# MingruiYuan/SpoofSV

Hardware: AMD Instinct MI355X
Metric: mel-frames/sec (Text2Mel+SSRN train) (higher is better)
Workload: dtype f32 (conv GEMMs: fp32 operands scaled by a power of two and split into fp16 hi+lo = 22 significand bits, three exact fp16 MFMAs per product, fp32 accumulate: ~2^-22 per product, gradients within 3e-6 of float64 = the exact-fp32 path's level); 1 GPU; train_text2mel + train_ssrn (train/ordinary.py step: fwd, l1+bin-div+guided-att losses, bwd, Adam), batch 32 utterances/GPU, N=186, T=325, 80 mel -> 513x1300 linear, hidden 256, random-init; global_batch=32, parallelism=dp1, launch=hipGraph replay, ddp=none

## Files before the change

### spoofsv_amd/csrc/api_conv.hip

```cpp
#include "ssv_host.h"

int conv_shifts(int k, int dilation, int causal, int* shift) {
  SSV_CHECK(k == 1 || k == 3, SSV_UNSUPPORTED, "conv1d: kernel_size %d not supported (1 or 3)", k);
  SSV_CHECK(dilation >= 1 && dilation * (k - 1) <= 54, SSV_UNSUPPORTED, "conv1d: dilation %d not supported (k=%d)", dilation, k);
  const int j0 = causal ? k - 1 : (k - 1) / 2;
  for (int j = 0; j < 3; ++j) shift[j] = j < k ? (j - j0) * dilation : 0;
  return 0;
}
extern "C" int ssv_conv_shifts(int k, int dilation, int causal, int* shift3) { return conv_shifts(k, dilation, causal, shift3); }

int amax_of(const float* x, long x_bs, int B, long n_item, const float* given, int ngiven, float* fb, AmaxList* out, hipStream_t st) {
  if (given) {
    SSV_CHECK(ngiven > 0, SSV_BAD_SHAPE, "operand scale list given with %d entries per item", ngiven);
    out->p = given; out->n = ngiven;
    return 0;
  }
  SSV_CHECK(fb, SSV_BAD_SHAPE, "split-fp16: no operand scales given and no workspace to compute them in");
  SSV_CHECK(B <= SSV_AMAX_FB_FLOATS, SSV_UNSUPPORTED, "split-fp16: batch %d needs caller-provided operand scales (ssv_absmax)", B);
  int npb = SSV_AMAX_FB_FLOATS / B;
  if (npb > 64) npb = 64;
  const long pieces = (n_item + 4095) / 4096;
  if (npb > pieces) npb = (int)(pieces > 0 ? pieces : 1);
  SSV_TRY(ssv_launch_absmax(x, x_bs, B, n_item, fb, npb, st));
  out->p = fb; out->n = npb;
// ... 194 lines not shown
  l.fb_dy = t.take(AMAX_FB_BYTES);
  l.fb_x = t.take(AMAX_FB_BYTES);
  l.total = t.off;
  return l;
}
extern "C" size_t ssv_conv1d_bwd_weight_workspace(int B, int Cin, int Cout, int L, int k) { return wgrad_ws(B, Cin, Cout, L, k).total; }
int conv1d_bwd_weight_impl(const float* dy, long dy_bs, const float* x, long x_bs, float* dw, int B, int Cin, int Cout, int L, int k, int dilation,
                           int causal, void* ws, size_t ws_bytes, ssv_stream_t stream, const float* part, float* pgrads, int n2, int nblk,
                           const float* dy_amax, int dy_namax, const float* x_amax, int x_namax) {
  SSV_CHECK(dy && x && dw && B > 0 && Cin > 0 && Cout > 0 && L > 0, SSV_BAD_SHAPE, "conv1d_bwd_weight: bad argument");
  const WgradWs l = wgrad_ws(B, Cin, Cout, L, k);
  SSV_CHECK(ws && ws_bytes >= l.total, SSV_BAD_SHAPE, "conv1d_bwd_weight: workspace too small");
  hipStream_t st = (hipStream_t)stream;
  GemmNT g;
  SSV_TRY(conv_shifts(k, dilation, causal, g.shift));
  int Z = l.Z;
  const float* slabs = ws_f32(ws, l.slabs);
  const long n = (long)Cout * Cin * k;
  g.A = dy; g.sab = dy_bs; g.sam = L; g.La = L;
  g.X = x; g.sxb = x_bs; g.sxc = L; g.Lx = L;
  g.M = Cout; g.Nc = Cin; g.KT = k; g.B = B;
  const bool bf3 = wgrad_bf3_runs(B, Cout, Cin, L, dy_bs, x_bs);
  if (!bf3 && Z > B) Z = B;
  if (Z == 1) { g.C = dw; g.scz = n; g.scm = (long)Cin * k; g.scc = k; g.scj = 1; }
  else { g.C = ws_f32(ws, l.slabs); g.scz = n; g.scm = (long)Cin * k; g.scc = 1; g.scj = Cin; }
  g.Z = Z; g.bstep = Z;
  if (bf3) {
    if (k != 3 && ssv_nt_bf3_xrow(1, Cout, Cin)) g.bstep = 0;
    if (use_f16()) {
      AmaxList la, lx;
      SSV_TRY(amax_of(dy, dy_bs, B, (long)Cout * L, dy_amax, dy_namax, ws_f32(ws, l.fb_dy), &la, st));
      SSV_TRY(amax_of(x, x_bs, B, (long)Cin * L, x_amax, x_namax, ws_f32(ws, l.fb_x), &lx, st));
      g.f16 = 1; g.a_amax = la.p; g.a_namax = la.n * B; g.x_amax = lx.p; g.x_namax = lx.n * B;
    }
    SSV_TRY(ssv_launch_gemm_nt_bf3(g, st));
  } else if (L == 1 && k == 1) {
    SSV_TRY(ssv_launch_linear_len1_wgrad(dy, dy_bs, x, x_bs, dw, B, Cin, Cout, st));
    if (part) SSV_TRY(ssv_reduce_partial_rows(part, pgrads, n2, nblk, st));
    return 0;
  } else SSV_TRY(ssv_launch_gemm_nt(g, st));
  if (part) {
    if (Z > 1 && nblk <= 768) return ssv_launch_reduce_pair(slabs, dw, Cout, Cin, k, Z, part, pgrads, n2, nblk, st);
    SSV_TRY(ssv_reduce_partial_rows(part, pgrads, n2, nblk, st));
  }
  if (Z > 1) SSV_TRY(ssv_launch_reduce_slabs_perm(slabs, dw, Cout, Cin, k, Z, st));
  return 0;
}
extern "C" int ssv_conv1d_bwd_weight(const float* dy, long dy_bs, const float* dy_amax, int dy_namax, const float* x, long x_bs, const float* x_amax, int x_namax,
                                     float* dw, int B, int Cin, int Cout, int L, int k, int dilation, int causal,
                                     void* ws, size_t ws_bytes, ssv_stream_t stream) {
  return conv1d_bwd_weight_impl(dy, dy_bs, x, x_bs, dw, B, Cin, Cout, L, k, dilation, causal, ws, ws_bytes, stream, nullptr, nullptr, 0, 0,
                                dy_amax, dy_namax, x_amax, x_namax);
}

extern "C" int ssv_conv1d_bwd_weight_multi_ok(int B, int Cin, int Cout, int L, int k) {
  return (k == 1 || k == 3) && L >= 8 && wgrad_bf3_runs_dense(B, Cout, Cin, L) ? 1 : 0;
}
extern "C" int ssv_conv1d_bwd_weight_multi_splits(int njobs, int B, int Cin, int Cout, int L, int k) {
  const int kt = k == 3 ? 3 : 1;
  if (njobs < 1) njobs = 1;
  const long tiles = (long)ssv_nt_bf3_tiles(kt, Cout, Cin) * njobs;
  if (kt == 1 && ssv_nt_bf3_xrow(1, Cout, Cin)) return xrow_slabs(tiles, B, L);
  int z = nt_slabs(tiles, njobs, B, L, kt, Cout, Cin);
  if (z > B) z = B;
  if (z < 1) z = 1;
  return z;
}
extern "C" size_t ssv_conv1d_bwd_weight_multi_workspace(int njobs, int B, int Cin, int Cout, int L, int k) {
  return align256((size_t)njobs * ssv_conv1d_bwd_weight_multi_splits(njobs, B, Cin, Cout, L, k) * Cout * Cin * k * sizeof(float));
}
extern "C" int ssv_conv1d_bwd_weight_multi(const ssv_wgrad_job* jobs_dev, int njobs, long dy_bs, long x_bs, int B, int Cin, int Cout, int L, int k, int max_shift,
                                           int n2, int nblk, void* ws, size_t ws_bytes, ssv_stream_t stream) {
  SSV_CHECK(jobs_dev && njobs > 0 && B > 0 && Cin > 0 && Cout > 0 && L > 0, SSV_BAD_SHAPE, "conv1d_bwd_weight_multi: bad argument");
  SSV_CHECK(ssv_conv1d_bwd_weight_multi_ok(B, Cin, Cout, L, k), SSV_UNSUPPORTED, "conv1d_bwd_weight_multi: shape or arithmetic mode not supported");
  SSV_CHECK(n2 == 0 || nblk <= 768, SSV_UNSUPPORTED, "conv1d_bwd_weight_multi: %d partial rows (max 768)", nblk);
  SSV_CHECK(ws && ws_bytes >= ssv_conv1d_bwd_weight_multi_workspace(njobs, B, Cin, Cout, L, k), SSV_BAD_SHAPE, "conv1d_bwd_weight_multi: workspace too small");
  hipStream_t st = (hipStream_t)stream;
  const int Z = ssv_conv1d_bwd_weight_multi_splits(njobs, B, Cin, Cout, L, k);
  const long n = (long)Cout * Cin * k;
  GemmNT g;
  g.sab = dy_bs; g.sam = L; g.La = L;
  g.sxb = x_bs; g.sxc = L; g.Lx = L;
  g.C = (float*)ws; g.scz = n; g.scm = (long)Cin * k; g.scc = 1; g.scj = Cin;
  g.M = Cout; g.Nc = Cin; g.KT = k; g.B = B; g.Z = Z; g.bstep = (k != 3 && ssv_nt_bf3_xrow(1, Cout, Cin)) ? 0 : Z;
  g.jobs = jobs_dev; g.njobs = njobs; g.max_shift = max_shift;
  g.f16 = use_f16() ? 1 : 0;
  SSV_TRY(ssv_launch_gemm_nt_bf3(g, st));
  return ssv_launch_reduce_pair_multi(jobs_dev, njobs, (const float*)ws, Cout, Cin, k, Z, n2, nblk, st);
}

static ConvWs deconv_fwd_ws(int Cin, int Cout) { return conv_ws(2 * split_bytes(Cout, Cin, 2)); }
extern "C" size_t ssv_deconv1d_k2s2_fwd_workspace(int Cin, int Cout) { return deconv_fwd_ws(Cin, Cout).total; }
extern "C" int ssv_deconv1d_k2s2_fwd(const float* x, long x_bs, const float* x_amax, int x_namax, const float* w, const void* w_packed, const float* bias,
                                     float* y, long y_bs, float* y_amax, int y_namax, int B, int Cin, int Cout, int L, void* ws, size_t ws_bytes, ssv_stream_t stream) {
  SSV_CHECK(x && w && y && B > 0 && Cin > 0 && Cout > 0 && L > 0, SSV_BAD_SHAPE, "deconv1d_k2s2_fwd: bad argument");
  SSV_CHECK(!y_amax || y_namax > 0, SSV_BAD_SHAPE, "deconv1d_k2s2_fwd: scale list of %d entries", y_namax);
  hipStream_t st = (hipStream_t)stream;
  if (use_bf3(B, L, Cin, Cout)) {
    const ConvWs l = deconv_fwd_ws(Cin, Cout);
    SSV_CHECK(ws && ws_bytes >= l.total, SSV_BAD_SHAPE, "deconv1d_k2s2_fwd: workspace too small");
    const int M2 = 2 * Cout, Kpad = pad32(Cin);
    const bool f16 = use_f16();
    float* aux = ws_f32(ws, l.aux);
    SplitPlanes pl = packed_planes(w_packed, Cin, M2, 1).tr;
    if (!pl.hi) {
      pl.hi = ws_u16(ws, l.main); pl.lo = ws_u16(ws, l.main + split_bytes(M2, Cin, 1));
      if (f16) { SSV_TRY(ssv_launch_pack_split_f16(w, (long)Cin * M2, pl.hi, pl.lo, M2, Cin, Kpad, 1, 1, (long)M2, 1, aux, st)); pl.inv = aux + 64; }
      else SSV_TRY(ssv_launch_pack_split(w, pl.hi, pl.lo, M2, Cin, Kpad, 1, 1, (long)M2, 1, 0, st));
    }
    GemmNNB g;
    if (f16) {
// ... 102 lines not shown
```

### spoofsv_amd/csrc/misc.hip

```cpp
#include "ssv_common.h"
#include "../../include/ssv_hip.h"

__global__ __launch_bounds__(256) void reduce_slabs_kernel(const float* __restrict__ s, float* __restrict__ out, long n, int Z, long stride) {
  const long i = (long)blockIdx.x * 256 + threadIdx.x;
  if (i >= n) return;
  float a[4] = {0.f, 0.f, 0.f, 0.f};
  int z = 0;
  for (; z + 3 < Z; z += 4) {
#pragma unroll
    for (int u = 0; u < 4; ++u) a[u] += s[(long)(z + u) * stride + i];
  }
  for (; z < Z; ++z) a[0] += s[(long)z * stride + i];
  out[i] = (a[0] + a[1]) + (a[2] + a[3]);
}
int ssv_launch_reduce_slabs(const float* slabs, float* out, long n, int Z, long stride, hipStream_t st) {
  hipLaunchKernelGGL(reduce_slabs_kernel, dim3(ssv_cdiv(n, 256)), dim3(256), 0, st, slabs, out, n, Z, stride);
  return ssv_check_launch("reduce_slabs");
}

__device__ __forceinline__ void reduce_perm_block(const float* __restrict__ s, float* __restrict__ out, int Nc, int KT, long n, int Z, int block,
                                                  float* __restrict__ stage ) {
  const long P = n / KT;
  const long q = (long)block * 256 + threadIdx.x;
  if (KT == 1) {
// ... 101 lines not shown
  __shared__ float red[8][32];
  const ssv_wgrad_job jb = jobs[blockIdx.y];
  const float* __restrict__ s = slabs + (long)blockIdx.y * Z * n;
  __shared__ __attribute__((aligned(16))) float stage[256 * 3];
  if ((int)blockIdx.x < nA) {
    reduce_perm_block(s, jb.dw, Nc, KT, n, Z, (int)blockIdx.x, stage);
    return;
  }
  if (!jb.part) return;
  const __attribute__((address_space(1))) float* __restrict__ part = (const __attribute__((address_space(1))) float*)jb.part;
  const int li = threadIdx.x & 31, rg = threadIdx.x >> 5;
  const int i = ((int)blockIdx.x - nA) * 32 + li;
  red[rg][li] = i < n2 ? ssv_fold_rows(part, n2, nblk, i, rg) : 0.f;
  __syncthreads();
  if (rg == 0 && i < n2) {
    float t = 0.f;
#pragma unroll
    for (int r = 0; r < 8; ++r) t += red[r][li];
    jb.pgrads[i] = t;
  }
}
int ssv_launch_reduce_pair_multi(const ssv_wgrad_job* jobs, int njobs, const float* slabs, int M, int Nc, int KT, int Z, int n2, int nblk, hipStream_t st) {
  const long n = (long)M * Nc * KT;
  const int nA = ssv_cdiv((long)M * Nc, 256), nB = n2 > 0 ? ssv_cdiv(n2, 32) : 0;
  hipLaunchKernelGGL(reduce_pair_multi_kernel, dim3(nA + nB, njobs), dim3(256), 0, st, jobs, slabs, Nc, KT, n, Z, nA, n2, nblk);
  return ssv_check_launch("reduce_pair_multi");
}

__global__ __launch_bounds__(256) void pack_wt_kernel(const float* __restrict__ w, float* __restrict__ wt, int Cout, int Cin, int KT) {
  const long i = (long)blockIdx.x * 256 + threadIdx.x;
  const long n = (long)Cout * Cin * KT;
  if (i >= n) return;
  const int j = (int)(i % KT);
  const long r = i / KT;
  const int o = (int)(r % Cout), c = (int)(r / Cout);
  wt[i] = w[((long)o * Cin + c) * KT + j];
}
int ssv_launch_pack_wt(const float* w, float* wt, int Cout, int Cin, int KT, hipStream_t st) {
  const long n = (long)Cout * Cin * KT;
  hipLaunchKernelGGL(pack_wt_kernel, dim3(ssv_cdiv(n, 256)), dim3(256), 0, st, w, wt, Cout, Cin, KT);
  return ssv_check_launch("pack_wt");
}

__global__ __launch_bounds__(256) void linear_len1_fwd_kernel(const float* __restrict__ x, long x_bs, const float* __restrict__ w, const float* __restrict__ bias,
                                                              const float* __restrict__ bias_b, long sbb, float* __restrict__ y, long y_bs, int B, int K, int M) {
  const long t = ((long)blockIdx.x * 256 + threadIdx.x) >> 3;
  const int j = threadIdx.x & 7;
// ... 579 lines not shown
```

### spoofsv_amd/csrc/ssv_common.h

```cpp
#pragma once
#include <hip/hip_runtime.h>
#include <stdint.h>
#include <stddef.h>
#include "../../include/ssv_hip.h"

int ssv_fail(int code, const char* fmt, ...);
#define SSV_BAD_SHAPE (-1)
#define SSV_UNSUPPORTED (-2)
#define SSV_CHECK(cond, code, ...) do { if (!(cond)) return ssv_fail((code), __VA_ARGS__); } while (0)
#define SSV_TRY(expr) do { int _e = (expr); if (_e) return _e; } while (0)
int ssv_check_launch(const char* what);

typedef __attribute__((ext_vector_type(4))) float f32x4;

struct GemmNN {
  const float* A = nullptr; long sab = 0, sam = 0, sac = 0, saj = 0;
  const float* X = nullptr; long sxb = 0, sxc = 0, sxn = 1; int Lx = 0;
  float* C = nullptr; long scb = 0, scm = 0, scn = 1;
  const float* bias = nullptr;
  const float* bias_b = nullptr; long sbb = 0;
  const float* R = nullptr; long srb = 0, srm = 0, srn = 1;
  int M = 0, N = 0, Kc = 0, KT = 1, B = 1;
  int shift[3] = {0, 0, 0};
  float alpha = 1.f;
// ... 21 lines not shown
  const float* R = nullptr; long srb = 0, srm = 0;
  int M = 0, N = 0, Kc = 0, KT = 1, B = 1;
  int shift[3] = {0, 0, 0};
  int sxn = 1, scn = 1;
  int row_pair = 0; float* c_amax = nullptr; int c_namax = 0;
  unsigned short* hs_planes = nullptr; long hs_plane_bytes = 0; int hs_npad = 0;
  int hs_keep_h = 1;
  int ksplit = 1; long scz = 0; int skip_rows = 0;
  const unsigned short* x0_planes = nullptr; const float* x0_amax = nullptr; int xsplit0 = 0;
  int perm_h = 0, epi = 0, first = 0;
  float* cstate = nullptr;
  float* lstm_out = nullptr; int lstm_s = 0, lstm_lo = 0, lstm_D = 0, xsplit = 0; long sab = 0;
  const unsigned short* A0hi = nullptr; const unsigned short* A0lo = nullptr;
  float* gates_out = nullptr;
  int f16 = 0; const float* a_inv = nullptr; const float* x_amax = nullptr; int x_namax = 0; long x_amax_bs = 0;
  float* colstats = nullptr;
  const float* xrow_w = nullptr; long xrow_sk = 0;
};
int ssv_launch_gemm_nn_bf3(const GemmNNB& g, hipStream_t st);
int ssv_launch_gemm_pwln(const GemmNNB& g, const float* gamma, const float* beta, float* y, long ybs, float* stats, float* y_amax, int namax, int act,
                         hipStream_t st);
int ssv_launch_gemm_nt_bf3(const GemmNT& g, hipStream_t st);
int ssv_launch_gemm_nt3r(const GemmNT& g, dim3 grid, int mtiles, int tchunks, int ring_ms, hipStream_t st);
struct PwLnBw {
  const float* dy; long dy_bs; const float* pre; const float* stats; const float* gamma; const float* beta;
  float* dpre; float* part; int part_rows; int part_q; float* amax; int namax;
  const unsigned short* Ahi; const unsigned short* Alo; const float* a_inv;
  float* dx; long dx_bs; const float* xrow_w; long xrow_sk;
  int M, Cin, L, act;
};
bool ssv_pwln_bwd_fused_ok(int B, int Cin, int Cout, int L);
int ssv_launch_pwln_bwd(const PwLnBw& q, int B, int f16, hipStream_t st);
bool ssv_nt_bf3_xrow(int KT, int M, int Nc);
bool ssv_nt_bf3_fits(const GemmNT& g);
int ssv_launch_pack_split(const float* w, void* hi, void* lo, int M, int K, int Kpad, int KT, long sm, long sk, long sj, int perm_h, hipStream_t st,
                          int nch_total = 0, int ch_off = 0);
int ssv_launch_pack_split_f16(const float* w, long w_elems, void* hi, void* lo, int M, int K, int Kpad, int KT, long sm, long sk, long sj, float* aux, hipStream_t st);
int ssv_launch_pack_split_f16_list(const float* w, void* hi, void* lo, int M, int K, int Kpad, int KT, long sm, long sk, long sj, int perm_h,
                                   const float* list, int nlist, float* inv_out, hipStream_t st, int nch_total = 0, int ch_off = 0);
#define SSV_F16_AUX_FLOATS 128
#define SSV_AMAX_FALLBACK 64
int ssv_launch_absmax(const float* x, long x_bs, int B, long n, float* out, int npb, hipStream_t st);
int ssv_nt_bf3_tiles(int KT, int M, int Nc);
void ssv_nt_bf3_tile(int KT, int M, int Nc, int* wm, int* ntc);
int ssv_nt_bf3_wg_per_cu(int KT, int wm, int ntc);
int ssv_precision();
// ... 97 lines not shown
```

### spoofsv_amd/csrc/wgrad_nt.hip

```cpp
#include "bf3_common.h"

#ifdef SSV_NT_STAMP
__device__ unsigned long long ssv_nt_stamps[64];
__device__ unsigned long long ssv_nt_wg[4096 * 4];
extern "C" int ssv_debug_nt_wg(unsigned long long* out) { return (int)hipMemcpyFromSymbol(out, HIP_SYMBOL(ssv_nt_wg), sizeof(ssv_nt_wg)); }
#define NT_WG(k, v) do { const unsigned w_ = blockIdx.z * gridDim.x + blockIdx.x; if (threadIdx.x == 0 && w_ < 4096u) ssv_nt_wg[w_ * 4 + (k)] = (v); } while (0)
#define NT_STAMP(k) do { if (stamp_on && (unsigned)(stamp_s - 24) < 8u) ssv_nt_stamps[(stamp_s - 24) * 8 + (k)] = __builtin_readcyclecounter(); } while (0)
extern "C" int ssv_debug_nt_stamps(unsigned long long* out) { return (int)hipMemcpyFromSymbol(out, HIP_SYMBOL(ssv_nt_stamps), sizeof(ssv_nt_stamps)); }
#else
#define NT_STAMP(k) do {} while (0)
#define NT_WG(k, v) do {} while (0)
#endif
constexpr int NT_FD = 1;
template <int KT, int WM, int NTC, int F16, int XR = 0, int WV = 4>
__global__ __launch_bounds__(64 * WV, WV == 4 ? 2 : 1) void gemm_nt_bf3_kernel(const GemmNT p, const int mtiles) {
  constexpr int NTH = 64 * WV;
  constexpr int KB = 64, KG = KB / 8, KS = KB / 32;
  constexpr int NCH = 16 * NTC;
  constexpr int X_SLOTS = KG * NCH;
  constexpr int NX = X_SLOTS / NTH;
  static_assert(X_SLOTS % NTH == 0, "tile slots must be a multiple of the workgroup size");
  __shared__ uint4 lds[2][2 * X_SLOTS];
  __shared__ float amax_sm[2 * WV];

// ... 353 lines not shown
}
int ssv_nt_bf3_wg_per_cu(int KT, int wm, int ntc) {
  if (wm == 4) return 1;
  if (KT == 3) return wm == 2 ? 2 : (ntc >= 4 ? 3 : 4);
  if (wm == 2) return ntc >= 6 ? 2 : 3;
  return ntc >= 6 ? 3 : (ntc >= 4 ? 4 : 5);
}
int ssv_nt_bf3_tiles(int KT, int M, int Nc) {
  int wm, ntc;
  ssv_nt_bf3_tile(KT, M, Nc, &wm, &ntc);
  return ssv_cdiv(ssv_nt_bf3_xrow(KT, M, Nc) ? M - 1 : M, 64 * wm) * ssv_cdiv(Nc, 16 * ntc);
}
bool ssv_nt_bf3_xrow(int KT, int M, int Nc) {
  int wm, ntc;
  ssv_nt_bf3_tile(KT, M, Nc, &wm, &ntc);
  return KT == 1 && wm == 2 && ntc == 6 && M > 128 && M % 128 == 1;
}

bool ssv_nt_bf3_fits(const GemmNT& g) {
  const long lim = 1L << 30;
  return (long)(g.B - 1) * g.sab + (long)(g.M - 1) * g.sam + g.La < lim && (long)(g.B - 1) * g.sxb + (long)(g.Nc - 1) * g.sxc + g.Lx < lim &&
         (long)g.B * g.sab < lim && (long)g.B * g.sxb < lim && g.La >= 8 && g.Lx >= 8;
}
int ssv_launch_gemm_nt_bf3(const GemmNT& g, hipStream_t st) {
  SSV_CHECK(g.M > 0 && g.Nc > 0 && g.La > 0 && g.B > 0 && g.Z > 0 && g.bstep >= 0, SSV_BAD_SHAPE, "gemm_nt_bf3: empty problem");
  SSV_CHECK(g.KT == 1 || g.KT == 3, SSV_UNSUPPORTED, "gemm_nt_bf3: kernel_size %d", g.KT);
  SSV_CHECK(g.sat == 1 && g.sxn == 1, SSV_UNSUPPORTED, "gemm_nt_bf3: rows must be contiguous in time");
  SSV_CHECK(g.Z <= 65535, SSV_UNSUPPORTED, "gemm_nt_bf3: Z=%d exceeds grid.z", g.Z);
  SSV_CHECK(ssv_nt_bf3_fits(g), SSV_UNSUPPORTED, "gemm_nt_bf3: an operand spans 2^30 elements or more");
  int wm, ntc;
  ssv_nt_bf3_tile(g.KT, g.M, g.Nc, &wm, &ntc);
  const bool xr = ssv_nt_bf3_xrow(g.KT, g.M, g.Nc);
  SSV_CHECK(g.bstep > 0 || xr, SSV_UNSUPPORTED, "gemm_nt_bf3: range slabs are built for the extra-row kernel only");
  const int mtiles = ssv_cdiv(xr ? g.M - 1 : g.M, 64 * wm);
  const int nz = g.jobs ? g.njobs * g.Z : g.Z;
  SSV_CHECK(nz <= 65535, SSV_UNSUPPORTED, "gemm_nt_bf3: %d slabs exceed grid.z", nz);
  const dim3 grid(mtiles * ssv_cdiv(g.Nc, 16 * ntc), 1, nz);
  SSV_CHECK(!g.f16 || g.jobs || (g.a_amax && g.x_amax && g.a_namax > 0 && g.x_namax > 0), SSV_BAD_SHAPE, "gemm_nt_bf3: split-fp16 needs both operand scales");
  int ring_ms = -1;
  if (g.KT == 3 && wm == 2 && ntc == 4) {
    ring_ms = g.max_shift;
    if (!g.jobs) { ring_ms = 0; for (int j = 0; j < 3; ++j) ring_ms = abs(g.shift[j]) > ring_ms ? abs(g.shift[j]) : ring_ms; }
    if (ring_ms > 64) ring_ms = -1;
  }
  if (ssv_shape_log_on()) {
    char nm[96], note[96];
    const int nj = g.jobs ? g.njobs : 1;
    if (ring_ms >= 0) snprintf(nm, sizeof nm, "gemm_nt3r_kernel<%d, %d>", wm, g.f16);
    else if (wm == 4) snprintf(nm, sizeof nm, "gemm_nt_bf3_kernel<%d, 2, %d, %d, 0, 8>", g.KT, ntc, g.f16);
    else snprintf(nm, sizeof nm, "gemm_nt_bf3_kernel<%d, %d, %d, %d, %d, 4>", g.KT, wm, ntc, g.f16, xr ? 1 : 0);
    snprintf(note, sizeof note, "jobs=%d B=%d M=%d Nc=%d L=%d k=%d Z=%d", nj, g.B, g.M, g.Nc, g.La, g.KT, g.Z);
    ssv_shape_log(nm, grid, dim3(wm == 4 ? 512 : 256), 2.0 * nj * g.B * g.M * g.Nc * g.La * g.KT,
                  4.0 * nj * ((double)g.B * g.M * g.La + (double)g.B * g.Nc * g.Lx + (double)g.Z * g.M * g.Nc * g.KT), note);
  }
  if (ring_ms >= 0) {
    const int tchunks = ssv_cdiv((g.La > g.Lx ? g.La : g.Lx) + ring_ms, 64);
    return ssv_launch_gemm_nt3r(g, grid, mtiles, tchunks, ring_ms, st);
  }
  if (xr) {
    if (g.f16) hipLaunchKernelGGL((gemm_nt_bf3_kernel<1, 2, 6, 1, 1>), grid, dim3(256), 0, st, g, mtiles);
    else hipLaunchKernelGGL((gemm_nt_bf3_kernel<1, 2, 6, 0, 1>), grid, dim3(256), 0, st, g, mtiles);
    return ssv_check_launch("gemm_nt_bf3 (extra row)");
  }
  if (g.KT == 1 && wm == 4 && ntc == 8) {
    if (g.f16) hipLaunchKernelGGL((gemm_nt_bf3_kernel<1, 2, 8, 1, 0, 8>), grid, dim3(512), 0, st, g, mtiles);
    else hipLaunchKernelGGL((gemm_nt_bf3_kernel<1, 2, 8, 0, 0, 8>), grid, dim3(512), 0, st, g, mtiles);
    return ssv_check_launch("gemm_nt_bf3 (8 waves)");
  }
#define SSV_NT(K_, A_, C_) if (g.KT == K_ && wm == A_ && ntc == C_) { \
    if (g.f16) hipLaunchKernelGGL((gemm_nt_bf3_kernel<K_, A_, C_, 1>), grid, dim3(256), 0, st, g, mtiles); \
    else hipLaunchKernelGGL((gemm_nt_bf3_kernel<K_, A_, C_, 0>), grid, dim3(256), 0, st, g, mtiles); \
    return ssv_check_launch("gemm_nt_bf3"); }
  SSV_NT(3, 2, 4)
  SSV_NT(1, 2, 8) SSV_NT(1, 2, 6) SSV_NT(1, 2, 2) SSV_NT(1, 1, 4)
#undef SSV_NT
  return ssv_fail(SSV_UNSUPPORTED, "gemm_nt_bf3: no tile %d,%d for kernel size %d", wm, ntc, g.KT);
// ... 3 lines not shown
```

### spoofsv_amd/csrc/wgrad_nt3r.hip

```cpp
#include "bf3_common.h"

#ifdef SSV_NT_STAMP
__device__ unsigned long long ssv_nt3r_stamps[64];
__device__ unsigned long long ssv_nt3r_wg[4096 * 4];
extern "C" int ssv_debug_nt3r_wg(unsigned long long* out) { return (int)hipMemcpyFromSymbol(out, HIP_SYMBOL(ssv_nt3r_wg), sizeof(ssv_nt3r_wg)); }
extern "C" int ssv_debug_nt3r_stamps(unsigned long long* out) { return (int)hipMemcpyFromSymbol(out, HIP_SYMBOL(ssv_nt3r_stamps), sizeof(ssv_nt3r_stamps)); }
#define NT_WG(k, v) do { const unsigned w_ = blockIdx.z * gridDim.x + blockIdx.x; if (threadIdx.x == 0 && w_ < 4096u) ssv_nt3r_wg[w_ * 4 + (k)] = (v); } while (0)
#define NT_STAMP(k) do { if (stamp_on && (unsigned)(stamp_s - 24) < 8u) ssv_nt3r_stamps[(stamp_s - 24) * 8 + (k)] = __builtin_readcyclecounter(); } while (0)
#else
#define NT_STAMP(k) do {} while (0)
#define NT_WG(k, v) do {} while (0)
#endif
typedef short ssv_s4 __attribute__((ext_vector_type(4)));
typedef __attribute__((address_space(3))) ssv_s4 ssv_lds_s4;
typedef unsigned ssv_u2 __attribute__((ext_vector_type(2)));
typedef __attribute__((address_space(3))) ssv_u2 ssv_lds_u2;
__device__ __forceinline__ void ssv_lds_store2(unsigned addr, unsigned a, unsigned b) {
#if defined(__HIP_DEVICE_COMPILE__)
  *(ssv_lds_u2*)(size_t)addr = (ssv_u2){a, b};
#else
  (void)addr; (void)a; (void)b;
#endif
}
__device__ __forceinline__ uint2 ssv_lds_read_tr16(unsigned addr) {
#if defined(__HIP_DEVICE_COMPILE__)
  return __builtin_bit_cast(uint2, __builtin_amdgcn_ds_read_tr16_b64_v4i16((ssv_lds_s4*)(size_t)addr));
#else
  (void)addr; return make_uint2(0u, 0u);
#endif
}
template <int WM, int F16>
__global__ __launch_bounds__(256, 2) void gemm_nt3r_kernel(const GemmNT p, const int mtiles, const int tchunks, const int max_shift) {
  constexpr int KT = 3, NTC = 4, NCH = 64, KB = 64, KS = 2;
  constexpr int R_FD = 1;
  constexpr unsigned ROWB = 128, PLANE = 288 * ROWB;
  __shared__ __attribute__((aligned(16))) unsigned char ring[2 * PLANE];
  __shared__ float amax_sm[8];

  const int tid = threadIdx.x, lane = tid & 63, wave = tid >> 6;
  NT_WG(0, __builtin_amdgcn_s_memrealtime()); NT_WG(2, __builtin_readcyclecounter());
  const unsigned wg = ssv_xcd_order(blockIdx.x + gridDim.x * blockIdx.z, gridDim.x * gridDim.z);
  const int bxx = (int)(wg % gridDim.x);
  int z = (int)(wg / gridDim.x);
  const float* __restrict__ Ap = p.A;
  const float* __restrict__ Xp = p.X;
  float* __restrict__ Cp = p.C;
  int shj[3] = {p.shift[0], p.shift[1], p.shift[2]};
  const float* __restrict__ a_amax = p.a_amax;
  const float* __restrict__ x_amax = p.x_amax;
  int a_namax = p.a_namax, x_namax = p.x_namax;
  if (p.jobs) {
    const int job = z / p.Z;
    z -= job * p.Z;
    const ssv_wgrad_job* __restrict__ jb = p.jobs + job;
    Ap = ssv_global(jb->dy); Xp = ssv_global(jb->x); Cp = p.C + (long)job * p.Z * p.scz;
    shj[0] = jb->shift[0]; shj[1] = jb->shift[1]; shj[2] = jb->shift[2];
    a_amax = ssv_global(jb->dy_amax); x_amax = ssv_global(jb->x_amax); a_namax = jb->dy_namax; x_namax = jb->x_namax;
  }
  float as = 1.f, xs = 1.f, us = 1.f;
  if constexpr (F16) {
    float sa, sx, ia, ix;
    ssv_pow2_scale(ssv_list_max<4>(a_amax, a_namax, amax_sm), sa, ia);
    ssv_pow2_scale(ssv_list_max<4>(x_amax, x_namax, amax_sm + 4), sx, ix);
    as = ssv_uniform(sa); xs = ssv_uniform(sx);
    us = ssv_uniform(ia * ix);
  }
  const int mt = bxx % mtiles, ct = bxx / mtiles;
  const int m0 = mt * 64 * WM, c0 = ct * NCH;
  const int kq = lane >> 4, nq = lane & 15;

  f32x4 acc[WM][KT][NTC];
#pragma unroll
  for (int i = 0; i < WM; ++i)
#pragma unroll
    for (int j = 0; j < KT; ++j)
#pragma unroll
      for (int q = 0; q < NTC; ++q) acc[i][j][q] = (f32x4){0.f, 0.f, 0.f, 0.f};

  uint4 AH[2][WM][KS], AL[2][WM][KS];
  uint4 rx[4];

  const __amdgpu_buffer_rsrc_t rsA = __builtin_amdgcn_make_buffer_rsrc(const_cast<float*>(Ap), 0,
      (int)(((long)(p.B - 1) * p.sab + (long)(p.M - 1) * p.sam + p.La) * 4), 0x00020000);
  const __amdgpu_buffer_rsrc_t rsX = __builtin_amdgcn_make_buffer_rsrc(const_cast<float*>(Xp), 0,
      (int)(((long)(p.B - 1) * p.sxb + (long)(p.Nc - 1) * p.sxc + p.Lx) * 4), 0x00020000);
  const unsigned arow = (unsigned)(((m0 + wave * WM * 16 + nq) * (int)p.sam + 4 * kq) * 4);
  const unsigned a16 = 16u * (unsigned)p.sam * 4u;
  const int cq = lane >> 4, tq = lane & 15;
  const unsigned xrow = (unsigned)(((c0 + 16 * wave + 4 * cq) * (int)p.sxc + 4 * tq) * 4);
  const unsigned x1 = (unsigned)p.sxc * 4u;
  const bool rows_in_c = c0 + NCH <= p.Nc;
  const unsigned ringb = (unsigned)(size_t)(__attribute__((address_space(3))) unsigned char*)ring;
  const unsigned waddr = ringb + (unsigned)(4 * tq) * ROWB + (unsigned)((wave ^ ((tq & 1) | (((tq >> 2) & 1) << 1))) << 5) + (unsigned)cq * 8u;
  const int q4 = (lane >> 2) & 3, pp = lane & 3;
  int lrow[2];
  lrow[0] = 4 * kq + (q4 >> 1) + 16 * (q4 & 1);
  lrow[1] = lrow[0] + 2;
  unsigned lbase[2], key5[KT][2];
#pragma unroll
  for (int r = 0; r < 2; ++r) {
    lbase[r] = ringb + (unsigned)lrow[r] * ROWB + (unsigned)pp * 8u;
#pragma unroll
    for (int j = 0; j < KT; ++j) { const int rr = shj[j] + lrow[r]; key5[j][r] = (unsigned)(((rr >> 2) & 1) | (((rr >> 4) & 1) << 1)) << 5; }
  }

  const int nb = (p.B - z + p.bstep - 1) / p.bstep;
  const int total = nb * tchunks;
  int cb[4], ct0[4];
  cb[0] = z; ct0[0] = 0;
  auto next_chunk = [&](int b, int t0, int& nb_, int& nt0) __attribute__((always_inline)) {
    nt0 = t0 + KB; nb_ = b;
    if (nt0 >= tchunks * KB) { nt0 = 0; nb_ = b + p.bstep; }
  };
#pragma unroll
  for (int k = 1; k < 4; ++k) next_chunk(cb[k - 1], ct0[k - 1], cb[k], ct0[k]);

  auto loadA = [&](auto set, int b, int t0) __attribute__((always_inline)) {
    constexpr int SET = decltype(set)::value;
    const unsigned so = ((unsigned)b * (unsigned)p.sab + (unsigned)t0) * 4u;
#pragma unroll
    for (int i = 0; i < WM; ++i)
#pragma unroll
      for (int s2 = 0; s2 < KS; ++s2) {
        AH[SET][i][s2] = __builtin_bit_cast(uint4, __builtin_amdgcn_raw_buffer_load_b128(rsA, (int)(arow + (so + i * a16)) + s2 * 128, 0, 0));
        AL[SET][i][s2] = __builtin_bit_cast(uint4, __builtin_amdgcn_raw_buffer_load_b128(rsA, (int)(arow + (so + i * a16)) + s2 * 128 + 64, 0, 0));
      }
  };
  auto loadA1 = [&](auto set, int b, int t0, int idx) __attribute__((always_inline)) {
    constexpr int SET = decltype(set)::value;
    const unsigned so = ((unsigned)b * (unsigned)p.sab + (unsigned)t0) * 4u;
// ... 70 lines not shown
    const int stamp_s = n + 16;
#endif
    NT_STAMP(0);
#pragma unroll
    for (int j = 0; j < KT; ++j) {
      constexpr int G = KS * NTC;
      uint4 fb[R_FD + 1][2];
      unsigned su[KS];
#pragma unroll
      for (int s2 = 0; s2 < KS; ++s2) su[s2] = (unsigned)((64 * n + shj[j] + 32 * s2) & 255) * ROWB;
      auto frag = [&](int g, uint4 (&f)[2]) __attribute__((always_inline)) {
        const int s2 = g / NTC, cbk = g % NTC;
        const unsigned a0 = lbase[0] + su[s2] + ((unsigned)(cbk << 5) ^ key5[j][0]);
        const unsigned a1 = lbase[1] + su[s2] + ((unsigned)(cbk << 5) ^ key5[j][1]);
        const uint2 h0u = ssv_lds_read_tr16(a0), h1u = ssv_lds_read_tr16(a1);
        const uint2 l0u = ssv_lds_read_tr16(a0 + PLANE), l1u = ssv_lds_read_tr16(a1 + PLANE);
        f[0] = make_uint4(h0u.x, h0u.y, h1u.x, h1u.y);
        f[1] = make_uint4(l0u.x, l0u.y, l1u.x, l1u.y);
      };
#pragma unroll
      for (int g = 0; g < R_FD; ++g) frag(g, fb[g]);
#pragma unroll
      for (int g = 0; g < G; ++g) {
        if (g + R_FD < G) frag(g + R_FD, fb[(g + R_FD) % (R_FD + 1)]);
        if (j == 0 && g < 4 * WM) loadA1(NXT{}, cb[1], ct0[1], g);
        if (j == 1 && g < 4) loadX1(cb[3], ct0[3], g);
        __builtin_amdgcn_sched_barrier(0);
        const int s2 = g / NTC, q = g % NTC;
        if (ct0[0] + 32 * s2 >= p.La) continue;
        const uint4 bh = fb[g % (R_FD + 1)][0];
        const uint4 bl = fb[g % (R_FD + 1)][1];
#pragma unroll
        for (int i = 0; i < WM; ++i) {
          const uint4 a_h = AH[CUR::value][i][s2];
          const uint4 a_l = AL[CUR::value][i][s2];
          acc[i][j][q] = mma16<F16>(a_l, bh, acc[i][j][q]);
          acc[i][j][q] = mma16<F16>(a_h, bl, acc[i][j][q]);
          acc[i][j][q] = mma16<F16>(a_h, bh, acc[i][j][q]);
        }
      }
      if (j == 0) {
        NT_STAMP(2);
        commitX((n + 2) & 3, ct0[2]);
        NT_STAMP(3);
      }
      if (j == 1) NT_STAMP(5);
// ... 4 lines not shown
      }
    }
    __syncthreads();
#pragma unroll
    for (int k = 0; k < 3; ++k) { cb[k] = cb[k + 1]; ct0[k] = ct0[k + 1]; }
    next_chunk(cb[2], ct0[2], cb[3], ct0[3]);
  };

  if (total > 0) {
    loadA(P0{}, cb[0], ct0[0]);
    loadX(cb[0], ct0[0]);
    {
#pragma unroll
      for (int i = 0; i < 4; ++i) {
        ssv_lds_store2(waddr + 3u * 64u * ROWB + i * ROWB, 0u, 0u);
        ssv_lds_store2(waddr + 3u * 64u * ROWB + i * ROWB + PLANE, 0u, 0u);
      }
    }
    commitX(0, ct0[0]);
    loadX(cb[1], ct0[1]);
    splitA(P0{}, ct0[0]);
    commitX(1, ct0[1]);
    loadX(cb[2], ct0[2]);
    __syncthreads();
    int n = 0;
    for (; n + 1 < total; n += 2) {
      chunk(P0{}, n);
      chunk(P1{}, n + 1);
    }
    if (n < total) chunk(P0{}, n);
  }

  NT_WG(3, __builtin_readcyclecounter());
  const bool bad_shift = abs(shj[0]) > max_shift || abs(shj[1]) > max_shift || abs(shj[2]) > max_shift;
  float* __restrict__ Cz = Cp + (long)z * p.scz;
#pragma unroll
  for (int i = 0; i < WM; ++i)
#pragma unroll
    for (int r = 0; r < 4; ++r) {
      const int gm = m0 + wave * WM * 16 + i * 16 + kq * 4 + r;
      if (gm >= p.M) continue;
#pragma unroll
      for (int j = 0; j < KT; ++j)
#pragma unroll
        for (int q = 0; q < NTC; ++q) {
          const int gc = c0 + q * 16 + nq;
          if (gc < p.Nc) Cz[(long)gm * p.scm + (long)gc * p.scc + (long)j * p.scj] = bad_shift ? __builtin_nanf("") : (F16 ? acc[i][j][q][r] * us : acc[i][j][q][r]);
        }
    }
#ifdef SSV_NT_STAMP
  __builtin_amdgcn_s_waitcnt(0);
#endif
  NT_WG(1, __builtin_amdgcn_s_memrealtime());
}


int ssv_launch_gemm_nt3r(const GemmNT& g, dim3 grid, int mtiles, int tchunks, int ring_ms, hipStream_t st) {
  if (g.f16) hipLaunchKernelGGL((gemm_nt3r_kernel<2, 1>), grid, dim3(256), 0, st, g, mtiles, tchunks, ring_ms);
  else hipLaunchKernelGGL((gemm_nt3r_kernel<2, 0>), grid, dim3(256), 0, st, g, mtiles, tchunks, ring_ms);
  return ssv_check_launch("gemm_nt3r");
}
```

Before: 852,100 mel-frames/s.

## Pair two batch slabs per nt3r workgroup and sum them in LDS before storing

The ring-buffered k=3 weight-gradient kernel now runs two 256-thread halves in one 512-thread workgroup, each processing a different batch slab. Their accumulators are exchanged through LDS and summed, so half as many slabs go to global memory. When only one paired slab remains in the multi-job path, the kernel writes dw directly and the reduction launch is skipped. The cost is a doubled LDS footprint with dynamic shared memory, one workgroup per CU, and extra barriers that keep the two halves in lockstep.

```diff
diff --git a/spoofsv_amd/csrc/api_conv.hip b/spoofsv_amd/csrc/api_conv.hip
--- a/spoofsv_amd/csrc/api_conv.hip
+++ b/spoofsv_amd/csrc/api_conv.hip
@@ -240,9 +240,10 @@
   g.M = Cout; g.Nc = Cin; g.KT = k; g.B = B;
   const bool bf3 = wgrad_bf3_runs(B, Cout, Cin, L, dy_bs, x_bs);
   if (!bf3 && Z > B) Z = B;
-  if (Z == 1) { g.C = dw; g.scz = n; g.scm = (long)Cin * k; g.scc = k; g.scj = 1; }
+  g.Z = Z; g.bstep = Z;
+  const int S = bf3 ? ssv_nt_bf3_slabs(g) : Z;
+  if (S == 1) { g.C = dw; g.scz = n; g.scm = (long)Cin * k; g.scc = k; g.scj = 1; }
   else { g.C = ws_f32(ws, l.slabs); g.scz = n; g.scm = (long)Cin * k; g.scc = 1; g.scj = Cin; }
-  g.Z = Z; g.bstep = Z;
   if (bf3) {
     if (k != 3 && ssv_nt_bf3_xrow(1, Cout, Cin)) g.bstep = 0;
     if (use_f16()) {
@@ -258,10 +259,10 @@
     return 0;
   } else SSV_TRY(ssv_launch_gemm_nt(g, st));
   if (part) {
-    if (Z > 1 && nblk <= 768) return ssv_launch_reduce_pair(slabs, dw, Cout, Cin, k, Z, part, pgrads, n2, nblk, st);
+    if (S > 1 && nblk <= 768) return ssv_launch_reduce_pair(slabs, dw, Cout, Cin, k, S, part, pgrads, n2, nblk, st);
     SSV_TRY(ssv_reduce_partial_rows(part, pgrads, n2, nblk, st));
   }
-  if (Z > 1) SSV_TRY(ssv_launch_reduce_slabs_perm(slabs, dw, Cout, Cin, k, Z, st));
+  if (S > 1) SSV_TRY(ssv_launch_reduce_slabs_perm(slabs, dw, Cout, Cin, k, S, st));
   return 0;
 }
 extern "C" int ssv_conv1d_bwd_weight(const float* dy, long dy_bs, const float* dy_amax, int dy_namax, const float* x, long x_bs, const float* x_amax, int x_namax,
@@ -303,8 +304,11 @@
   g.M = Cout; g.Nc = Cin; g.KT = k; g.B = B; g.Z = Z; g.bstep = (k != 3 && ssv_nt_bf3_xrow(1, Cout, Cin)) ? 0 : Z;
   g.jobs = jobs_dev; g.njobs = njobs; g.max_shift = max_shift;
   g.f16 = use_f16() ? 1 : 0;
+  int S = ssv_nt_bf3_slabs(g);
+  if (ssv_nt_ring_bound(g) >= 0 && S == 1) { g.C = nullptr; g.scm = (long)Cin * k; g.scc = k; g.scj = 1; S = 0; }
   SSV_TRY(ssv_launch_gemm_nt_bf3(g, st));
-  return ssv_launch_reduce_pair_multi(jobs_dev, njobs, (const float*)ws, Cout, Cin, k, Z, n2, nblk, st);
+  if (S == 0 && n2 == 0) return 0;
+  return ssv_launch_reduce_pair_multi(jobs_dev, njobs, (const float*)ws, Cout, Cin, k, S, n2, nblk, st);
 }
 
 static ConvWs deconv_fwd_ws(int Cin, int Cout) { return conv_ws(2 * split_bytes(Cout, Cin, 2)); }
diff --git a/spoofsv_amd/csrc/misc.hip b/spoofsv_amd/csrc/misc.hip
--- a/spoofsv_amd/csrc/misc.hip
+++ b/spoofsv_amd/csrc/misc.hip
@@ -147,7 +147,8 @@
 }
 int ssv_launch_reduce_pair_multi(const ssv_wgrad_job* jobs, int njobs, const float* slabs, int M, int Nc, int KT, int Z, int n2, int nblk, hipStream_t st) {
   const long n = (long)M * Nc * KT;
-  const int nA = ssv_cdiv((long)M * Nc, 256), nB = n2 > 0 ? ssv_cdiv(n2, 32) : 0;
+  const int nA = Z > 0 ? ssv_cdiv((long)M * Nc, 256) : 0, nB = n2 > 0 ? ssv_cdiv(n2, 32) : 0;
+  if (nA + nB == 0) return 0;
   hipLaunchKernelGGL(reduce_pair_multi_kernel, dim3(nA + nB, njobs), dim3(256), 0, st, jobs, slabs, Nc, KT, n, Z, nA, n2, nblk);
   return ssv_check_launch("reduce_pair_multi");
 }
diff --git a/spoofsv_amd/csrc/ssv_common.h b/spoofsv_amd/csrc/ssv_common.h
--- a/spoofsv_amd/csrc/ssv_common.h
+++ b/spoofsv_amd/csrc/ssv_common.h
@@ -67,6 +67,8 @@
                          hipStream_t st);
 int ssv_launch_gemm_nt_bf3(const GemmNT& g, hipStream_t st);
 int ssv_launch_gemm_nt3r(const GemmNT& g, dim3 grid, int mtiles, int tchunks, int ring_ms, hipStream_t st);
+int ssv_nt_ring_bound(const GemmNT& g);
+int ssv_nt_bf3_slabs(const GemmNT& g);
 struct PwLnBw {
   const float* dy; long dy_bs; const float* pre; const float* stats; const float* gamma; const float* beta;
   float* dpre; float* part; int part_rows; int part_q; float* amax; int namax;
diff --git a/spoofsv_amd/csrc/wgrad_nt.hip b/spoofsv_amd/csrc/wgrad_nt.hip
--- a/spoofsv_amd/csrc/wgrad_nt.hip
+++ b/spoofsv_amd/csrc/wgrad_nt.hip
@@ -399,6 +399,15 @@
   return (long)(g.B - 1) * g.sab + (long)(g.M - 1) * g.sam + g.La < lim && (long)(g.B - 1) * g.sxb + (long)(g.Nc - 1) * g.sxc + g.Lx < lim &&
          (long)g.B * g.sab < lim && (long)g.B * g.sxb < lim && g.La >= 8 && g.Lx >= 8;
 }
+int ssv_nt_ring_bound(const GemmNT& g) {
+  int wm, ntc;
+  ssv_nt_bf3_tile(g.KT, g.M, g.Nc, &wm, &ntc);
+  if (!(g.KT == 3 && wm == 2 && ntc == 4)) return -1;
+  int ms = g.max_shift;
+  if (!g.jobs) { ms = 0; for (int j = 0; j < 3; ++j) ms = abs(g.shift[j]) > ms ? abs(g.shift[j]) : ms; }
+  return ms > 64 ? -1 : ms;
+}
+int ssv_nt_bf3_slabs(const GemmNT& g) { return ssv_nt_ring_bound(g) >= 0 ? (g.Z + 1) / 2 : g.Z; }
 int ssv_launch_gemm_nt_bf3(const GemmNT& g, hipStream_t st) {
   SSV_CHECK(g.M > 0 && g.Nc > 0 && g.La > 0 && g.B > 0 && g.Z > 0 && g.bstep >= 0, SSV_BAD_SHAPE, "gemm_nt_bf3: empty problem");
   SSV_CHECK(g.KT == 1 || g.KT == 3, SSV_UNSUPPORTED, "gemm_nt_bf3: kernel_size %d", g.KT);
@@ -410,16 +419,12 @@
   const bool xr = ssv_nt_bf3_xrow(g.KT, g.M, g.Nc);
   SSV_CHECK(g.bstep > 0 || xr, SSV_UNSUPPORTED, "gemm_nt_bf3: range slabs are built for the extra-row kernel only");
   const int mtiles = ssv_cdiv(xr ? g.M - 1 : g.M, 64 * wm);
-  const int nz = g.jobs ? g.njobs * g.Z : g.Z;
+  const int ring_ms = ssv_nt_ring_bound(g);
+  const int nslabs = ssv_nt_bf3_slabs(g);
+  const int nz = g.jobs ? g.njobs * nslabs : nslabs;
   SSV_CHECK(nz <= 65535, SSV_UNSUPPORTED, "gemm_nt_bf3: %d slabs exceed grid.z", nz);
   const dim3 grid(mtiles * ssv_cdiv(g.Nc, 16 * ntc), 1, nz);
   SSV_CHECK(!g.f16 || g.jobs || (g.a_amax && g.x_amax && g.a_namax > 0 && g.x_namax > 0), SSV_BAD_SHAPE, "gemm_nt_bf3: split-fp16 needs both operand scales");
-  int ring_ms = -1;
-  if (g.KT == 3 && wm == 2 && ntc == 4) {
-    ring_ms = g.max_shift;
-    if (!g.jobs) { ring_ms = 0; for (int j = 0; j < 3; ++j) ring_ms = abs(g.shift[j]) > ring_ms ? abs(g.shift[j]) : ring_ms; }
-    if (ring_ms > 64) ring_ms = -1;
-  }
   if (ssv_shape_log_on()) {
     char nm[96], note[96];
     const int nj = g.jobs ? g.njobs : 1;
@@ -427,8 +432,8 @@
     else if (wm == 4) snprintf(nm, sizeof nm, "gemm_nt_bf3_kernel<%d, 2, %d, %d, 0, 8>", g.KT, ntc, g.f16);
     else snprintf(nm, sizeof nm, "gemm_nt_bf3_kernel<%d, %d, %d, %d, %d, 4>", g.KT, wm, ntc, g.f16, xr ? 1 : 0);
     snprintf(note, sizeof note, "jobs=%d B=%d M=%d Nc=%d L=%d k=%d Z=%d", nj, g.B, g.M, g.Nc, g.La, g.KT, g.Z);
-    ssv_shape_log(nm, grid, dim3(wm == 4 ? 512 : 256), 2.0 * nj * g.B * g.M * g.Nc * g.La * g.KT,
-                  4.0 * nj * ((double)g.B * g.M * g.La + (double)g.B * g.Nc * g.Lx + (double)g.Z * g.M * g.Nc * g.KT), note);
+    ssv_shape_log(nm, grid, dim3(wm == 4 || ring_ms >= 0 ? 512 : 256), 2.0 * nj * g.B * g.M * g.Nc * g.La * g.KT,
+                  4.0 * nj * ((double)g.B * g.M * g.La + (double)g.B * g.Nc * g.Lx + (double)nslabs * g.M * g.Nc * g.KT), note);
   }
   if (ring_ms >= 0) {
     const int tchunks = ssv_cdiv((g.La > g.Lx ? g.La : g.Lx) + ring_ms, 64);
diff --git a/spoofsv_amd/csrc/wgrad_nt3r.hip b/spoofsv_amd/csrc/wgrad_nt3r.hip
--- a/spoofsv_amd/csrc/wgrad_nt3r.hip
+++ b/spoofsv_amd/csrc/wgrad_nt3r.hip
@@ -1,4 +1,5 @@
 #include "bf3_common.h"
+#include <atomic>
 
 #ifdef SSV_NT_STAMP
 __device__ unsigned long long ssv_nt3r_stamps[64];
@@ -29,19 +30,39 @@
   (void)addr; return make_uint2(0u, 0u);
 #endif
 }
+typedef __attribute__((address_space(3))) f32x4 ssv_lds_f4;
+__device__ __forceinline__ void ssv_lds_store_f4(unsigned addr, f32x4 v) {
+#if defined(__HIP_DEVICE_COMPILE__)
+  *(ssv_lds_f4*)(size_t)addr = v;
+#else
+  (void)addr; (void)v;
+#endif
+}
+__device__ __forceinline__ f32x4 ssv_lds_load_f4(unsigned addr) {
+#if defined(__HIP_DEVICE_COMPILE__)
+  return *(ssv_lds_f4*)(size_t)addr;
+#else
+  (void)addr; return (f32x4){0.f, 0.f, 0.f, 0.f};
+#endif
+}
+constexpr unsigned NT3R_PLANE = 288u * 128u;
+constexpr unsigned NT3R_LDS = 4u * NT3R_PLANE + 16u * sizeof(float);
 template <int WM, int F16>
-__global__ __launch_bounds__(256, 2) void gemm_nt3r_kernel(const GemmNT p, const int mtiles, const int tchunks, const int max_shift) {
+__global__ __launch_bounds__(512, 1) void gemm_nt3r_kernel(const GemmNT p, const int mtiles, const int tchunks, const int max_shift) {
+  static_assert(WM == 2, "the pair sum exchanges one of two row blocks");
   constexpr int KT = 3, NTC = 4, NCH = 64, KB = 64, KS = 2;
   constexpr int R_FD = 1;
-  constexpr unsigned ROWB = 128, PLANE = 288 * ROWB;
-  __shared__ __attribute__((aligned(16))) unsigned char ring[2 * PLANE];
-  __shared__ float amax_sm[8];
-
-  const int tid = threadIdx.x, lane = tid & 63, wave = tid >> 6;
+  constexpr unsigned ROWB = 128, PLANE = NT3R_PLANE;
+  extern __shared__ __attribute__((aligned(16))) unsigned char nt3r_lds[];
+  float* amax_sm = reinterpret_cast<float*>(nt3r_lds + 4 * PLANE);
+
+  const int tid = threadIdx.x, lane = tid & 63, wave = (tid >> 6) & 3;
+  const int half = __builtin_amdgcn_readfirstlane(tid >> 8);
   NT_WG(0, __builtin_amdgcn_s_memrealtime()); NT_WG(2, __builtin_readcyclecounter());
   const unsigned wg = ssv_xcd_order(blockIdx.x + gridDim.x * blockIdx.z, gridDim.x * gridDim.z);
   const int bxx = (int)(wg % gridDim.x);
-  int z = (int)(wg / gridDim.x);
+  int pq = (int)(wg / gridDim.x);
+  const int npairs = (p.Z + 1) >> 1;
   const float* __restrict__ Ap = p.A;
   const float* __restrict__ Xp = p.X;
   float* __restrict__ Cp = p.C;
@@ -50,18 +71,19 @@
   const float* __restrict__ x_amax = p.x_amax;
   int a_namax = p.a_namax, x_namax = p.x_namax;
   if (p.jobs) {
-    const int job = z / p.Z;
-    z -= job * p.Z;
+    const int job = pq / npairs;
+    pq -= job * npairs;
     const ssv_wgrad_job* __restrict__ jb = p.jobs + job;
-    Ap = ssv_global(jb->dy); Xp = ssv_global(jb->x); Cp = p.C + (long)job * p.Z * p.scz;
+    Ap = ssv_global(jb->dy); Xp = ssv_global(jb->x);
+    Cp = p.C ? p.C + (long)job * npairs * p.scz : ssv_global(jb->dw);
     shj[0] = jb->shift[0]; shj[1] = jb->shift[1]; shj[2] = jb->shift[2];
     a_amax = ssv_global(jb->dy_amax); x_amax = ssv_global(jb->x_amax); a_namax = jb->dy_namax; x_namax = jb->x_namax;
   }
   float as = 1.f, xs = 1.f, us = 1.f;
   if constexpr (F16) {
     float sa, sx, ia, ix;
-    ssv_pow2_scale(ssv_list_max<4>(a_amax, a_namax, amax_sm), sa, ia);
-    ssv_pow2_scale(ssv_list_max<4>(x_amax, x_namax, amax_sm + 4), sx, ix);
+    ssv_pow2_scale(ssv_list_max<8>(a_amax, a_namax, amax_sm), sa, ia);
+    ssv_pow2_scale(ssv_list_max<8>(x_amax, x_namax, amax_sm + 8), sx, ix);
     as = ssv_uniform(sa); xs = ssv_uniform(sx);
     us = ssv_uniform(ia * ix);
   }
@@ -90,7 +112,8 @@
   const unsigned xrow = (unsigned)(((c0 + 16 * wave + 4 * cq) * (int)p.sxc + 4 * tq) * 4);
   const unsigned x1 = (unsigned)p.sxc * 4u;
   const bool rows_in_c = c0 + NCH <= p.Nc;
-  const unsigned ringb = (unsigned)(size_t)(__attribute__((address_space(3))) unsigned char*)ring;
+  const unsigned ldsb = (unsigned)(size_t)(__attribute__((address_space(3))) unsigned char*)nt3r_lds;
+  const unsigned ringb = ldsb + (unsigned)half * (2u * PLANE);
   const unsigned waddr = ringb + (unsigned)(4 * tq) * ROWB + (unsigned)((wave ^ ((tq & 1) | (((tq >> 2) & 1) << 1))) << 5) + (unsigned)cq * 8u;
   const int q4 = (lane >> 2) & 3, pp = lane & 3;
   int lrow[2];
@@ -104,8 +127,11 @@
     for (int j = 0; j < KT; ++j) { const int rr = shj[j] + lrow[r]; key5[j][r] = (unsigned)(((rr >> 2) & 1) | (((rr >> 4) & 1) << 1)) << 5; }
   }
 
-  const int nb = (p.B - z + p.bstep - 1) / p.bstep;
-  const int total = nb * tchunks;
+  const int z = 2 * pq + half;
+  auto chunks_of = [&](int zz) __attribute__((always_inline)) { return zz < p.Z ? ((p.B - zz + p.bstep - 1) / p.bstep) * tchunks : 0; };
+  const int tot0 = chunks_of(2 * pq), tot1 = chunks_of(2 * pq + 1);
+  const int total = half ? tot1 : tot0;
+  const int iters = tot0 > tot1 ? tot0 : tot1;
   int cb[4], ct0[4];
   cb[0] = z; ct0[0] = 0;
   auto next_chunk = [&](int b, int t0, int& nb_, int& nt0) __attribute__((always_inline)) {
@@ -222,6 +248,7 @@
       for (int g = 0; g < R_FD; ++g) frag(g, fb[g]);
 #pragma unroll
       for (int g = 0; g < G; ++g) {
+        if (j == 1 && g == G / 2) __builtin_amdgcn_s_barrier();
         if (g + R_FD < G) frag(g + R_FD, fb[(g + R_FD) % (R_FD + 1)]);
         if (j == 0 && g < 4 * WM) loadA1(NXT{}, cb[1], ct0[1], g);
         if (j == 1 && g < 4) loadX1(cb[3], ct0[3], g);
@@ -272,32 +299,57 @@
     splitA(P0{}, ct0[0]);
     commitX(1, ct0[1]);
     loadX(cb[2], ct0[2]);
-    __syncthreads();
+  }
+  __syncthreads();
+  if (half) __builtin_amdgcn_s_barrier();
+  {
     int n = 0;
     for (; n + 1 < total; n += 2) {
       chunk(P0{}, n);
       chunk(P1{}, n + 1);
     }
-    if (n < total) chunk(P0{}, n);
-  }
+    if (n < total) { chunk(P0{}, n); ++n; }
+    for (; n < iters; ++n) { __builtin_amdgcn_s_barrier(); __syncthreads(); }
+  }
+  const unsigned park_mine = ringb + (unsigned)wave * (12u * 64u * 16u) + (unsigned)lane * 16u;
+  const unsigned park_other = park_mine + (half ? 0u - 2u * PLANE : 2u * PLANE);
+  auto park = [&](auto blk) __attribute__((always_inline)) {
+    constexpr int I = decltype(blk)::value;
+#pragma unroll
+    for (int j = 0; j < KT; ++j)
+#pragma unroll
+      for (int q = 0; q < NTC; ++q) ssv_lds_store_f4(park_mine + (unsigned)(j * NTC + q) * 1024u, acc[I][j][q]);
+  };
+  if (half == 0) { park(P1{}); __builtin_amdgcn_s_barrier(); }
+  else park(P0{});
 
   NT_WG(3, __builtin_readcyclecounter());
   const bool bad_shift = abs(shj[0]) > max_shift || abs(shj[1]) > max_shift || abs(shj[2]) > max_shift;
-  float* __restrict__ Cz = Cp + (long)z * p.scz;
-#pragma unroll
-  for (int i = 0; i < WM; ++i)
+  float* __restrict__ Cz = Cp + (long)pq * p.scz;
+  auto add_store = [&](auto blk) __attribute__((always_inline)) {
+    constexpr int I = decltype(blk)::value;
+#pragma unroll
+    for (int j = 0; j < KT; ++j)
+#pragma unroll
+      for (int q = 0; q < NTC; ++q) {
+        const f32x4 o = ssv_lds_load_f4(park_other + (unsigned)(j * NTC + q) * 1024u);
+        acc[I][j][q] = I == 0 ? acc[I][j][q] + o : o + acc[I][j][q];
+      }
 #pragma unroll
     for (int r = 0; r < 4; ++r) {
-      const int gm = m0 + wave * WM * 16 + i * 16 + kq * 4 + r;
+      const int gm = m0 + wave * WM * 16 + I * 16 + kq * 4 + r;
       if (gm >= p.M) continue;
 #pragma unroll
       for (int j = 0; j < KT; ++j)
 #pragma unroll
         for (int q = 0; q < NTC; ++q) {
           const int gc = c0 + q * 16 + nq;
-          if (gc < p.Nc) Cz[(long)gm * p.scm + (long)gc * p.scc + (long)j * p.scj] = bad_shift ? __builtin_nanf("") : (F16 ? acc[i][j][q][r] * us : acc[i][j][q][r]);
+          if (gc < p.Nc) Cz[(long)gm * p.scm + (long)gc * p.scc + (long)j * p.scj] = bad_shift ? __builtin_nanf("") : (F16 ? acc[I][j][q][r] * us : acc[I][j][q][r]);
         }
     }
+  };
+  __syncthreads();
+  if (half == 0) add_store(P0{}); else add_store(P1{});
 #ifdef SSV_NT_STAMP
   __builtin_amdgcn_s_waitcnt(0);
 #endif
@@ -305,8 +357,24 @@
 }
 
 
+static int nt3r_lds_limit() {
+  static std::atomic<int> done[64];
+  int dev = 0;
+  hipError_t e = hipGetDevice(&dev);
+  if (e != hipSuccess) return ssv_fail(-(int)e, "gemm_nt3r: hipGetDevice: %s", hipGetErrorString(e));
+  if (dev >= 0 && dev < 64 && done[dev].load(std::memory_order_acquire)) return 0;
+  const void* ks[2] = {(const void*)gemm_nt3r_kernel<2, 1>, (const void*)gemm_nt3r_kernel<2, 0>};
+  for (int i = 0; i < 2; ++i) {
+    e = hipFuncSetAttribute(ks[i], hipFuncAttributeMaxDynamicSharedMemorySize, (int)NT3R_LDS);
+    if (e != hipSuccess) return ssv_fail(-(int)e, "gemm_nt3r: hipFuncSetAttribute(MaxDynamicSharedMemorySize): %s", hipGetErrorString(e));
+  }
+  if (dev >= 0 && dev < 64) done[dev].store(1, std::memory_order_release);
+  return 0;
+}
 int ssv_launch_gemm_nt3r(const GemmNT& g, dim3 grid, int mtiles, int tchunks, int ring_ms, hipStream_t st) {
-  if (g.f16) hipLaunchKernelGGL((gemm_nt3r_kernel<2, 1>), grid, dim3(256), 0, st, g, mtiles, tchunks, ring_ms);
-  else hipLaunchKernelGGL((gemm_nt3r_kernel<2, 0>), grid, dim3(256), 0, st, g, mtiles, tchunks, ring_ms);
+  SSV_CHECK(g.bstep == g.Z && (g.C || (g.jobs && g.Z <= 2)), SSV_BAD_SHAPE, "gemm_nt3r: whole-item ranges and an output");
+  SSV_TRY(nt3r_lds_limit());
+  if (g.f16) hipLaunchKernelGGL((gemm_nt3r_kernel<2, 1>), grid, dim3(512), NT3R_LDS, st, g, mtiles, tchunks, ring_ms);
+  else hipLaunchKernelGGL((gemm_nt3r_kernel<2, 0>), grid, dim3(512), NT3R_LDS, st, g, mtiles, tchunks, ring_ms);
   return ssv_check_launch("gemm_nt3r");
 }
```

Result: no change. 856,700 mel-frames/s, median of 6 (+0.5%).
